# NidhiMishra/SR_object_detection

Hardware: AMD Instinct MI355X
Metric: images/sec YOLOv2 608x608 fp32 (higher is better)
Workload: dtype f32

## Files before the change

### include/y2_hip.h

```cpp
#ifndef Y2_HIP_H
#define Y2_HIP_H

#include <stddef.h>
#include <stdint.h>

#ifdef __cplusplus
extern "C" {
#endif

#define Y2H_OK            0
#define Y2H_EHIP         -1
#define Y2H_EINVAL       -2
#define Y2H_ENODEV       -3

typedef void *y2h_stream;
typedef void *y2h_event;
typedef void *y2h_graph;

enum { Y2H_ACT_LINEAR = 0, Y2H_ACT_LEAKY = 1, Y2H_ACT_LOGISTIC = 2, Y2H_ACT_RELU = 3,
       Y2H_ACT_RELIE = 4, Y2H_ACT_RAMP = 5, Y2H_ACT_TANH = 6, Y2H_ACT_PLSE = 7, Y2H_ACT_ELU = 8, Y2H_ACT_LOGGY = 9,
       Y2H_ACT_STAIR = 10, Y2H_ACT_HARDTAN = 11, Y2H_ACT_LHTAN = 12 };

int         y2h_device_count(void);
int         y2h_set_device(int dev);
// ... 49 lines not shown
    int activation;
    const float  *x;
    const float  *w_packed;
    const float  *w_ref;
    const float  *mean;
    const double *rinv;
    const float  *scale;
    const float  *bias;
    float        *y;
    float        *ws;
    size_t        ws_bytes;
    int           x_f16;
    int           y_f16;
    const float  *alpha;
    const float  *beta;
    int           tile_bm, tile_bn;
    int           ksplit;
    int           x_nchw;
} y2h_conv;

int y2h_conv_candidates(const y2h_conv *d, int *bm, int *bn, int *ks, int max);

int y2h_conv_first_layer_nchw_ok(const y2h_conv *d);

int y2h_conv_uses_mfma(const y2h_conv *d);
size_t y2h_conv_workspace_bytes(const y2h_conv *d);
int y2h_p8_stream_k_plan(long ntiles, int nk, long grid, int *sk_tiles, int *sk_wgs);
int y2h_sk_shares(long tiles, int nk, long G, int *out);
int y2h_sk_first(long tiles, int nk, long G, int *out);
int y2h_sk_walk(long tiles, int nk, long G, int *out, int max);
unsigned long y2h_stream_k_launches(void);
unsigned long y2h_tail_launches(void);
unsigned long y2h_xcd_order_launches(void);
unsigned long y2h_f32_stream_k_launches(void);
int y2h_conv_first_layer_ok(const y2h_conv *d);
int y2h_conv_stem_halo(const y2h_conv *d);
int y2h_conv_first_layer_f16_ok(const y2h_conv *d);
int y2h_conv_forward(const y2h_conv *d, int strict, y2h_stream s);
const char *y2h_conv_variant(const y2h_conv *d, int strict);

typedef struct y2h_wino {
    int eligible;
    int take;
    int bm, bn;
    long tiles, tiles_pad;
    size_t u_bytes;
    size_t v_bytes, m_bytes;
    double direct_cost, gemm_cost, wino_cost;
} y2h_wino;
int y2h_wino_plan(const y2h_conv *d, y2h_wino *out);
size_t y2h_wino_workspace_bytes(const y2h_conv *d);
int y2h_conv_wino_forward(const y2h_conv *d, y2h_stream s);
unsigned long y2h_wino_launches(void);

int y2h_maxpool(const float *x, int ldx, float *y, int ldy, int batch, int h, int w, int c,
                int size, int stride, int pad, int out_h, int out_w, y2h_stream s);
int y2h_reorg(const float *x, int ldx, float *y, int ldy, int batch, int h, int w, int c,
              int stride, int reverse, y2h_stream s);
int y2h_connected_ref(const float *x, long x_batch_stride, int ld, int hw, int c, const float *w_ref, float *y,
                      int outputs, int batch, int batch_normalize, int activation, const float *mean,
                      const double *rinv, const float *scale, const float *bias, y2h_stream s);
int y2h_detection_boxes(const float *pred, long pred_stride, int batch, int side, int num, int classes, int sqrt_flag,
                        int w, int h, float thresh, int only_objectness, float *boxes, float *probs, y2h_stream s);
int y2h_shortcut(const float *in, int ld_in, const float *add, int ld_add, float *out, int ld_out, int batch,
                 int w1, int h1, int c1, int w2, int h2, int c2, int activation, y2h_stream s);
int y2h_crop(const float *x, int ldx, float *y, int ldy, int batch, int h, int w, int c, int out_h, int out_w,
             int noadjust, int halo, y2h_stream s);
int y2h_batchnorm(const float *x, int ldx, float *y, int ldy, long pixels, int c, const float *mean, const double *rinv,
                  const float *scale, y2h_stream s);
int y2h_local(const float *x, int ldx, const float *w_packed, const float *bias_packed, float *y, int ldy, int batch,
              int h, int w, int c, int n, int size, int stride, int pad, int out_h, int out_w, int activation,
              int strict, y2h_stream s);
int y2h_binarize(const float *x, int ldx, float *y, long rows, int c, y2h_stream s);
int y2h_activate_array(float *x, int ld, long rows, int c, int activation, y2h_stream s);
int y2h_activate_copy(const float *x, int ldx, float *y, int ldy, long rows, int c, int activation, y2h_stream s);
int y2h_activate_copy_f16(const void *x, int ldx, void *y, int ldy, long rows, int c, int activation, y2h_stream s);
int y2h_lrn_fast_ok(int c, int size);
int y2h_lrn(const float *x, int ldx, float *y, int ldy, long pixels, int c, int size, float alpha, float beta, float kappa,
            int strict, y2h_stream s);
int y2h_lrn_f16(const void *x, int ldx, void *y, int ldy, long pixels, int c, int size, float alpha, float beta, float kappa,
                y2h_stream s);
int y2h_avgpool(const float *x, int ldx, float *y, int batch, int h, int w, int c, y2h_stream s);
int y2h_softmax_rows(const float *x, float *y, long rows, int n, float temp, y2h_stream s);
int y2h_softmax_tree_rows(const float *x, float *y, long rows, int n, float temp, int groups, const int *group_size,
                          const int *group_offset, const int *group_of, y2h_stream s);
int y2h_hierarchy_rows(float *rows, long ld, int nrows, int n, const int *parent, const int *order, const int *level_off,
                       int levels, const int *leaf, const int *row_mask, y2h_stream s);

int y2h_maxpool_f16(const void *x, int ldx, void *y, int ldy, int batch, int h, int w, int c,
                    int size, int stride, int pad, int out_h, int out_w, y2h_stream s);
int y2h_reorg_f16(const void *x, int ldx, void *y, int ldy, int batch, int h, int w, int c,
                  int stride, int reverse, y2h_stream s);
int y2h_copy_channels_f16(const void *src, int ld_src, void *dst, int ld_dst, int c, long npix, y2h_stream s);
int y2h_avgpool_f16(const void *x, int ldx, float *y, int batch, int h, int w, int c, y2h_stream s);
int y2h_nhwc_f16_to_nchw(const void *src, int ld, float *dst, int n, int c, int h, int w, y2h_stream s);
int y2h_nchw_to_nhwc4_halo_f16(const float *src, void *dst, int n, int c, int h, int w, y2h_stream s);
int y2h_f32_to_f16(const float *src, void *dst, long n, y2h_stream s);
int y2h_f16_to_f32(const void *src, float *dst, long n, y2h_stream s);

int y2h_connected_f16_plan(int rows, int inputs, int outputs, int forced, int *ranges, size_t *ws_bytes, int *bounds,
                           int max_bounds);
int y2h_connected_f16(const void *x, long ldx, const void *w, const float *alpha, const float *beta, void *y, int ldy,
                      int y_f16, int rows, int inputs, int outputs, int activation, int ranges, float *ws, size_t ws_bytes,
                      y2h_stream s);
int y2h_local_f16(const void *x, int ldx, const void *w_packed, const float *bias_packed, void *y, int ldy, int batch,
                  int h, int w, int c, int n, int size, int stride, int pad, int out_h, int out_w, int activation,
// ... 228 lines not shown
```

### sr_object_detection_amd/csrc/host/y2_arena.c

```c
#include <math.h>
#include <stdio.h>
#include <stdlib.h>
#include <string.h>
#include "y2_internal.h"
#include "y2_wino_rule.h"

static int owns_arena(const layer *l)
{
    return l->type == CONVOLUTIONAL || l->type == CONNECTED || l->type == LOCAL || l->type == BATCHNORM || is_recurrent(l);
}

void y2_bn_slots(size_t *off, int n, size_t *mean, size_t *scale, size_t *rinv)
{
    *mean = *off; *off = align_up(*off + n * sizeof(float), 64);
    *scale = *off; *off = align_up(*off + n * sizeof(float), 64);
    *rinv = *off; *off = align_up(*off + n * sizeof(double), 64);
}

void y2_fill_rinv(double *dst, const float *var, int n)
{
    int f;
    for (f = 0; f < n; ++f) dst[f] = 1.0 / (sqrt((double)var[f]) + (double).000001f);
}

static float xnor_filter_mean(const float *w, int K)
{
    float bmean = 0;
    int q;
    for (q = 0; q < K; ++q) bmean += fabs(w[q]);
    return bmean / K;
}

static unsigned short f32_to_f16_rne(float f)
{
    unsigned int x, sign, mant;
    int exp;
    memcpy(&x, &f, sizeof x);
    sign = (x >> 16) & 0x8000u;
    exp = (int)((x >> 23) & 0xff) - 127 + 15;
    mant = x & 0x7fffffu;
    if (((x >> 23) & 0xff) == 0xff) return (unsigned short)(sign | 0x7c00u | (mant ? 0x200u : 0));
    if (exp >= 31) return (unsigned short)(sign | 0x7c00u);
    if (exp <= 0) {
        unsigned int shift, half, rem;
        if (exp < -10) return (unsigned short)sign;
        mant |= 0x800000u;
        shift = (unsigned int)(14 - exp);
        half = mant >> shift;
        rem = mant & ((1u << shift) - 1);
        if (rem > (1u << (shift - 1)) || (rem == (1u << (shift - 1)) && (half & 1))) ++half;
        return (unsigned short)(sign | half);
    }
    {
        unsigned int half = ((unsigned int)exp << 10) | (mant >> 13), rem = mant & 0x1fffu;
        if (rem > 0x1000u || (rem == 0x1000u && (half & 1))) ++half;
        return (unsigned short)(sign | half);
    }
}

void y2_arena_layout(network *net)
{
    y2_engine *e = y2_engine_of(net);
    size_t off = 0;
    int i;
    for (i = 0; i < net->n; ++i) {
        const layer *l = &net->layers[i];
        y2_ldev *d = ld_of(l);
        const size_t wbytes = (size_t)l->n * l->size * l->size * l->c * sizeof(float);
        const int w_half = y2_half_weights(net, i);
        if (!owns_arena(l)) continue;
        if (l->type == BATCHNORM) { y2_bn_slots(&off, l->c, &d->off_mean, &d->off_scale, &d->off_rinv); continue; }
        if (is_recurrent(l)) { off = y2_rec_layout(d, l, off); continue; }
        if (l->type == LOCAL) {
            d->off_w_packed = off; off = align_up(off + (size_t)l->out_h * l->out_w * l->n * l->size * l->size * l->c * (w_half ? 2 : sizeof(float)), 256);
            d->off_bias = off; off = align_up(off + (size_t)l->outputs * sizeof(float), 64);
            continue;
        }
        d->off_w_packed = off; off = align_up(off + (d->wino ? (size_t)16 * l->n * l->c * sizeof(float) : w_half ? wbytes / 2 : wbytes), 256);
        if (d->has_w_ref) { d->off_w_ref = off; off = align_up(off + wbytes, 256); }
        d->off_bias = off; off = align_up(off + l->n * sizeof(float), 64);
        if (w_half) {
            d->off_alpha = off; off = align_up(off + l->n * sizeof(float), 64);
            d->off_beta = off; off = align_up(off + l->n * sizeof(float), 64);
        }
        if (l->batch_normalize) y2_bn_slots(&off, l->n, &d->off_mean, &d->off_scale, &d->off_rinv);
    }
    e->arena_need = off;
}

static uint64_t arena_signature(const network *net)
{
    const y2_engine *e = y2_engine_of(net);
    uint64_t sig = 1469598103934665603ull;
    int i, k;
#define SIG_MIX(v) do { uint64_t v_ = (uint64_t)(v); int b_; for (b_ = 0; b_ < 8; ++b_) { sig ^= (v_ >> (8 * b_)) & 0xff; sig *= 1099511628211ull; } } while (0)
    for (i = 0; i < net->n; ++i) {
        const layer *l = &net->layers[i];
        const y2_ldev *d = ld_of(l);
        if (!owns_arena(l)) continue;
        if (is_recurrent(l)) {
            for (k = 0; k < 3; ++k) { SIG_MIX(i); SIG_MIX(d->rd[k].off_w); SIG_MIX(d->rd[k].off_bias); SIG_MIX(d->rd[k].bn ? d->rd[k].off_rinv + 1 : 0); }
            continue;
        }
        SIG_MIX(i); SIG_MIX(d->off_w_packed); SIG_MIX(d->has_w_ref ? d->off_w_ref + 1 : 0); SIG_MIX(d->off_bias);
        SIG_MIX(d->uses_mfma); SIG_MIX(y2_half_weights(net, i));
        SIG_MIX(l->batch_normalize ? d->off_rinv + 1 : 0);
        if (d->wino) SIG_MIX(0x57494e4f);
    }
    SIG_MIX(e->strict); SIG_MIX(e->half); SIG_MIX(e->arena_need);
#undef SIG_MIX
    return sig;
}

int y2_arena_commit(network *net)
{
    y2_engine *e = y2_engine_of(net);
    const uint64_t sig = arena_signature(net);
    const int had_layout = e->arena_sig != 0;
    if (e->arena_need != e->arena_bytes || !e->arena) {
        if (e->arena) y2h_free(e->arena);
        e->arena = NULL;
        e->arena_bytes = e->arena_need;
        HIP_OR_ERR(y2h_malloc((void **)&e->arena, e->arena_need));
        e->arena_sig = 0;
    }
    if (sig == e->arena_sig) return 0;
    if (e->weights_external && had_layout) {
        e->weights_external = 0;
        y2_fail("the weight arena was filled from outside (y2_weights_resident) for another plan "
                "(strict / fp16 / fusion / size changed its layout): call y2_weights_arena() again and replicate the "
                "weights for the new plan");
        return -1;
    }
    if (!e->weights_external) e->weights_dirty = 1;
    e->arena_sig = sig;
    return 0;
}

static void pack_local(unsigned char *host, const y2_ldev *d, const layer *l, int w_half)
{
    const int locations = l->out_h * l->out_w, kk = l->size * l->size, K = kk * l->c;
    float *wp = (float *)(host + d->off_w_packed), *b = (float *)(host + d->off_bias);
    int loc, co, ci, t;
    for (loc = 0; loc < locations; ++loc)
        for (co = 0; co < l->n; ++co) {
            const float *src = l->weights + ((size_t)loc * l->n + co) * K;
            float *dst = wp + ((size_t)loc * l->n + co) * K;
            for (ci = 0; ci < l->c; ++ci)
                for (t = 0; t < kk; ++t) {
                    if (w_half) ((unsigned short *)wp)[((size_t)loc * l->n + co) * K + (size_t)t * l->c + ci] = f32_to_f16_rne(src[(size_t)ci * kk + t]);
                    else dst[(size_t)t * l->c + ci] = src[(size_t)ci * kk + t];
                }
            b[(size_t)loc * l->n + co] = l->biases[(size_t)co * locations + loc];
        }
}

static void pack_filters(float *wp, const network *net, int i, int w_half)
{
    const layer *l = &net->layers[i];
    const int K = l->size * l->size * l->c;
    int co, ci, kh, kw;
    if (l->type == CONNECTED) {
        const layer *pl = i > 0 ? &net->layers[y2_producer_of(net, i)] : NULL;
        const int hw = (pl && !y2_is_flat(net, y2_producer_of(net, i))) ? pl->out_h * pl->out_w : 1;
        const int C = K / (hw > 0 ? hw : 1);
        int pix;
        for (co = 0; co < l->n; ++co)
            for (ci = 0; ci < C; ++ci)
                for (pix = 0; pix < hw; ++pix) {
                    const size_t dst = (size_t)co * K + (size_t)pix * C + ci;
                    const float v = l->weights[(size_t)co * K + (size_t)ci * hw + pix];
                    if (w_half) ((unsigned short *)wp)[dst] = f32_to_f16_rne(v);
                    else wp[dst] = v;
                }
        return;
    }
    for (co = 0; co < l->n; ++co) {
        const float bmean = l->xnor ? xnor_filter_mean(l->weights + (size_t)co * K, K) : 0;
        for (ci = 0; ci < l->c; ++ci)
            for (kh = 0; kh < l->size; ++kh)
                for (kw = 0; kw < l->size; ++kw) {
                    const size_t dst = (size_t)co * K + (size_t)(kh * l->size + kw) * l->c + ci;
                    float v = l->weights[(((size_t)co * l->c + ci) * l->size + kh) * l->size + kw];
                    if (l->xnor) v = (v > 0) ? bmean : -bmean;
                    if (w_half) ((unsigned short *)wp)[dst] = f32_to_f16_rne(v);
                    else wp[dst] = v;
                }
    }
}

static void pack_wino(float *up, const layer *l)
{
    const size_t comp = (size_t)l->n * l->c;
    int co, ci, g;
    for (co = 0; co < l->n; ++co)
        for (ci = 0; ci < l->c; ++ci) {
            float u[16];
            y2_wino_filter(l->weights + ((size_t)co * l->c + ci) * 9, u);
            for (g = 0; g < 16; ++g) up[g * comp + (size_t)co * l->c + ci] = u[g];
        }
}

static void pack_dense(unsigned char *host, const network *net, int i)
{
    const layer *l = &net->layers[i];
    const y2_ldev *d = ld_of(l);
    const int K = l->size * l->size * l->c, w_half = y2_half_weights(net, i);
    int co, f, q;
    if (d->wino) pack_wino((float *)(host + d->off_w_packed), l);
    else pack_filters((float *)(host + d->off_w_packed), net, i, w_half);
    if (w_half) {
        float *al = (float *)(host + d->off_alpha), *be = (float *)(host + d->off_beta);
        for (f = 0; f < l->n; ++f) {
            double a = 1.0, bb = l->biases[f];
            if (l->batch_normalize) {
                a = (double)l->scales[f] / (sqrt((double)l->rolling_variance[f]) + (double).000001f);
                bb = (double)l->biases[f] - (double)l->rolling_mean[f] * a;
            }
            al[f] = (float)a; be[f] = (float)bb;
        }
    }
    if (d->has_w_ref) memcpy(host + d->off_w_ref, l->weights, (size_t)l->n * K * sizeof(float));
    if (d->has_w_ref && l->type == CONVOLUTIONAL && l->xnor) {
        float *wr = (float *)(host + d->off_w_ref);
        for (co = 0; co < l->n; ++co) {
            const float bmean = xnor_filter_mean(l->weights + (size_t)co * K, K);
            for (q = 0; q < K; ++q) wr[(size_t)co * K + q] = (l->weights[(size_t)co * K + q] > 0) ? bmean : -bmean;
        }
    }
    memcpy(host + d->off_bias, l->biases, l->n * sizeof(float));
    if (l->batch_normalize) {
        memcpy(host + d->off_mean, l->rolling_mean, l->n * sizeof(float));
        memcpy(host + d->off_scale, l->scales, l->n * sizeof(float));
        y2_fill_rinv((double *)(host + d->off_rinv), l->rolling_variance, l->n);
    }
}

int y2_upload_weights(network *net)
{
    y2_engine *e = y2_engine_of(net);
    unsigned char *host = NULL;
    int i;
    if (y2h_host_alloc((void **)&host, e->arena_bytes ? e->arena_bytes : 16) != 0) host = NULL;
    if (!host) { y2_fail("weight upload: no pinned host memory for %zu bytes: %s", e->arena_bytes, y2h_last_error()); return -1; }
    memset(host, 0, e->arena_bytes ? e->arena_bytes : 16);
    for (i = 0; i < net->n; ++i) {
        const layer *l = &net->layers[i];
        const y2_ldev *d = ld_of(l);
        if (!owns_arena(l)) continue;
        if (is_recurrent(l)) y2_rec_pack(host, d, l);
        else if (l->type == BATCHNORM) {
            memcpy(host + d->off_mean, l->rolling_mean, l->c * sizeof(float));
            memcpy(host + d->off_scale, l->scales, l->c * sizeof(float));
            y2_fill_rinv((double *)(host + d->off_rinv), l->rolling_variance, l->c);
        }
        else if (l->type == LOCAL) pack_local(host, d, l, y2_half_weights(net, i));
        else pack_dense(host, net, i);
    }
    if (y2h_memcpy_h2d(e->arena, host, e->arena_bytes, e->stream) != 0 || y2h_stream_sync(e->stream) != 0) {
        y2h_host_free(host);
        y2_fail("weight upload failed: %s", y2h_last_error());
        return -1;
// ... 37 lines not shown
```

### sr_object_detection_amd/csrc/host/y2_engine.c

```c
#include <math.h>
#include <stdio.h>
#include <stdlib.h>
#include <string.h>
#include "y2_internal.h"

void y2_drop_graphs(y2_engine *e)
{
    int k;
    for (k = 0; k < 4; ++k) {
        if (e->graphs[k]) y2h_graph_destroy(e->graphs[k]);
        e->graphs[k] = NULL; e->graph_srcs[k] = NULL;
    }
    e->graph = NULL; e->graph_src = NULL; e->graph_next = 0;
}

y2_engine *y2_engine_of(const network *net) { return net ? (y2_engine *)net->engine : NULL; }

int y2_engine_create(network *net)
{
    y2_engine *e = calloc(1, sizeof *e);
    int i;
    const char *st = getenv("Y2_STRICT");
    e->device = net->gpu_index;
    e->weights_dirty = 1;
// ... 142 lines not shown
    return 0;
}

static int forward_input(network *net, const float *d_input_nchw)
{
    y2_engine *e = y2_engine_of(net);
    const int misaligned = ((uintptr_t)d_input_nchw % 16) != 0;
    e->cur_input = d_input_nchw;
    if (y2_flat_input(net)) {
        if (misaligned && d_input_nchw != e->d_in_nchw) {
            HIP_OR_ERR(y2h_memcpy_d2d(e->d_in_nchw, d_input_nchw, e->in_floats * sizeof(float), e->stream));
            e->cur_input = e->d_in_nchw;
        }
        return 0;
    }
    switch (e->in_form) {
    case Y2_IN_NCHW:
        if (!e->half || !misaligned) break;
        if (d_input_nchw != e->d_in_nchw) HIP_OR_ERR(y2h_memcpy_d2d(e->d_in_nchw, d_input_nchw, e->in_floats * sizeof(float), e->stream));
        e->cur_input = e->d_in_nchw;
        break;
    case Y2_IN_NHWC4_HALO_F16:
        HIP_OR_ERR(y2h_nchw_to_nhwc4_halo_f16(d_input_nchw, e->d_in_nhwc, net->batch, net->c, net->h, net->w, e->stream));
        break;
    case Y2_IN_NHWC_HALO:
        HIP_OR_ERR(y2h_nchw_to_nhwc_halo(d_input_nchw, e->d_in_nhwc, net->batch, net->c, net->h, net->w, net->c, e->in_halo_px, e->stream));
        break;
    case Y2_IN_NHWC:
        HIP_OR_ERR(y2h_nchw_to_nhwc(d_input_nchw, e->d_in_nhwc, net->batch, net->c, net->h, net->w, net->c, e->stream));
        break;
    }
    return 0;
}

int y2_activate_after(y2_engine *e, ACTIVATION a, float *y, int ld, long rows, int n)
{
    if (!y2_act_in_kernel(a)) HIP_OR_ERR(y2h_activate_array(y, ld, rows, n, y2_act_code(a), e->stream));
    return 0;
}

static int forward_convolutional(network *net, int i, const float *x, int ldx)
{
    y2_engine *e = y2_engine_of(net);
    const layer *l = &net->layers[i];
    const y2_ldev *d = ld_of(l);
    y2h_conv c;
    if (l->xnor) {
        const float *px; int pld;
        if (i == 0) { px = e->d_in_nhwc; pld = net->c; }
        else { const y2_ldev *p = ld_of(&net->layers[i - 1]); px = p->out; pld = p->out_ld; }
        HIP_OR_ERR(y2h_binarize(px, pld, d->d_bin, (long)l->batch * l->h * l->w, l->c, e->stream));
    }
    y2_conv_desc(net, i, &c, x, ldx);
    if (d->wino) HIP_OR_ERR(y2h_conv_wino_forward(&c, e->stream));
    else HIP_OR_ERR(y2h_conv_forward(&c, e->strict, e->stream));
    return y2_activate_after(e, l->activation, d->out, d->out_ld, (long)l->batch * l->out_h * l->out_w, l->out_c);
}

static int forward_route(network *net, int i)
{
    y2_engine *e = y2_engine_of(net);
    const layer *l = &net->layers[i];
    const y2_ldev *d = ld_of(l);
    int k, choff = 0;
    if (l->n < 2 || !d->copy_mask) return 0;
    for (k = 0; k < l->n; ++k) {
        const layer *src = &net->layers[l->input_layers[k]];
        const y2_ldev *sd = ld_of(src);
        if ((d->copy_mask & (1u << k)) && d->out_half)
            HIP_OR_ERR(y2h_copy_channels_f16(sd->out, sd->out_ld, (unsigned short *)d->out + choff, d->out_ld, src->out_c,
                                             (long)l->batch * l->out_h * l->out_w, e->stream));
        else if (d->copy_mask & (1u << k))
            HIP_OR_ERR(y2h_copy_channels(sd->out, sd->out_ld, d->out + choff, d->out_ld, src->out_c,
                                         (long)l->batch * l->out_h * l->out_w, e->stream));
        choff += src->out_c;
    }
    return 0;
}

static int forward_region(network *net, int i, const float *x, int ldx)
{
    y2_engine *e = y2_engine_of(net);
    const layer *l = &net->layers[i];
    y2_ldev *d = ld_of(l);
    const tree *t = l->softmax_tree;
    if (e->det_overlap && e->det_pending == 1 && i == e->out_layer && !e->capturing) HIP_OR_ERR(y2h_stream_wait_event(e->stream, e->ev_det));
    d->tree_best_valid = 0;
    if (t && d->d_tree_best && !e->det_overlap) d->tree_best_valid = 1;
    if (t)
        HIP_OR_ERR(y2h_region_forward_tree(x, ldx, d->d_region, l->batch, l->h * l->w, l->n, l->classes, l->coords, t->groups,
                                           d->d_tree_gsize, d->d_tree_goff, d->d_tree_parent, d->d_tree_order, d->d_tree_loff,
                                           d->tree_levels, d->tree_best_valid ? d->d_tree_best : NULL,
                                           e->strict ? 0 : Y2H_REGION_FAST_EXP, e->stream));
    else
        HIP_OR_ERR(y2h_region_forward(x, ldx, d->d_region, l->batch, l->h * l->w, l->n, l->classes, l->coords, l->softmax,
                                      0, d->d_tree_gsize, d->d_tree_goff, e->stream));
    return 0;
}

static int forward_connected(network *net, int i, const float *x, int ldx)
{
    y2_engine *e = y2_engine_of(net);
    const layer *l = &net->layers[i];
    const y2_ldev *d = ld_of(l);
    y2h_conv c;
    y2_conv_desc(net, i, &c, x, ldx);
    if (d->conn_ranges && !e->strict) {
// ... 548 lines not shown
```

### sr_object_detection_amd/csrc/host/y2_internal.h

```cpp
#ifndef Y2_INTERNAL_H
#define Y2_INTERNAL_H

#include <stddef.h>
#include <stdint.h>
#include "sr_yolo2.h"
#include "y2_hip.h"

typedef struct y2_ldev {
    struct y2_engine *eng;
    int index;
    float *out;
    int out_ld;
    float *out_alloc;
    size_t out_floats;
    int placed_in;
    int alias_of;
    unsigned copy_mask;
    size_t off_w_packed, off_w_ref, off_bias, off_mean, off_scale, off_rinv;
    int has_w_ref;
    int uses_mfma;
    int wino;
    int fused_pool;
    int fused_into;
    int out_half;
    size_t off_alpha, off_beta;
    char kname[80];
    int tile_bm, tile_bn, ksplit;
    int conn_ranges;
    float *d_anchors;
    int *d_tree_block, *h_tree_block;
    size_t tree_block_ints;
    int *d_tree_parent, *d_tree_gsize, *d_tree_goff, *d_map;
    int *d_tree_order, *d_tree_loff;
    int tree_levels;
    int *d_tree_group, *d_tree_leaf, *h_tree_leaf;
    float *d_tree_best;
    int tree_best_valid;
    float *d_region;
    float *d_flat;
    float *d_halo;
    int halo_px;
    float *d_bin;
    const char *kernel;
    struct { size_t off_w, off_bias, off_mean, off_scale, off_rinv; int n, k, bn; ACTIVATION act; int form; } rd[3];
    float *d_state;
    float *d_proj;
    float *d_hist;
    float *d_zf;
    float *d_tmp;
} y2_ldev;

enum { Y2_REC_REF = 0, Y2_REC_SKINNY = 1, Y2_REC_MFMA = 2 };

enum { Y2_LR_CONSTANT = 0, Y2_LR_STEP, Y2_LR_EXP, Y2_LR_POLY, Y2_LR_STEPS, Y2_LR_SIG, Y2_LR_RANDOM };
typedef struct {
    int policy, step, burn_in, num_steps, adam;
    float scale, gamma, power;
    int *steps;
    float *scales;
} y2_lr_schedule;

typedef struct y2_engine {
    int device;
    y2h_stream stream;
    int strict;
    int timing;
    int fusion, built_fusion;
    int half, built_half;
    int autotune, built_autotune;
    int in_form;
    const float *cur_input;
    int in_halo_px;
    y2h_event ev_out;
    int out_pending;
// ... 163 lines not shown
```

### sr_object_detection_amd/csrc/host/y2_plan.c

```c
#include <math.h>
#include <stdio.h>
#include <stdlib.h>
#include <pthread.h>
#include <string.h>
#include "y2_internal.h"

void y2_free_plan(network *net)
{
    y2_engine *e = y2_engine_of(net);
    int i;
    if (!e) return;
    for (i = 0; i < net->n; ++i) {
        y2_ldev *d = ld_of(&net->layers[i]);
        if (!d) continue;
        y2h_free(d->out_alloc); d->out_alloc = NULL; d->out = NULL;
        y2h_free(d->d_region); d->d_region = NULL;
        y2h_free(d->d_flat); d->d_flat = NULL;
        y2h_free(d->d_halo); d->d_halo = NULL; d->halo_px = 0;
        y2h_free(d->d_bin); d->d_bin = NULL;
        y2h_free(d->d_state); d->d_state = NULL;
        y2h_free(d->d_proj); d->d_proj = NULL;
        y2h_free(d->d_hist); d->d_hist = NULL;
        y2h_free(d->d_zf); d->d_zf = NULL;
        y2h_free(d->d_tmp); d->d_tmp = NULL;
        d->placed_in = -1; d->alias_of = -1; d->copy_mask = 0;
        d->fused_pool = 0; d->fused_into = -1;
        d->out_half = 0;
        d->wino = 0;
        d->tile_bm = d->tile_bn = d->ksplit = 0;
        d->conn_ranges = 0;
    }
    y2_drop_graphs(e);
    y2h_free(e->d_in_nchw); e->d_in_nchw = NULL;
    y2h_free(e->d_in_nhwc); e->d_in_nhwc = NULL;
    y2h_free(e->d_out_nchw); e->d_out_nchw = NULL;
    y2h_free(e->d_ws); e->d_ws = NULL; e->ws_bytes = 0;
    y2h_free(e->d_u8); e->d_u8 = NULL; e->u8_cap = 0;
    y2h_free(e->d_planes); e->d_planes = NULL; e->planes_cap = 0;
    y2h_free(e->d_rtmp); e->d_rtmp = NULL; e->rtmp_cap = 0;
    if (e->reg_pending) { y2h_event_sync(e->ev_reg); e->reg_pending = 0; }
    y2h_free(e->d_reg); e->d_reg = NULL; e->reg_cap = 0;
    y2h_free(e->d_boxes); e->d_boxes = NULL;
    y2h_free(e->d_probs); e->d_probs = NULL;
    y2h_free(e->d_probs_nms); e->d_probs_nms = NULL;
    y2h_free(e->d_records); e->d_records = NULL;
    y2h_free(e->d_counts); e->d_counts = NULL;
    y2h_free(e->d_class_counts); e->d_class_counts = NULL;
    y2h_free(e->d_best); e->d_best = NULL;
    y2h_free(e->d_mean_ring); e->d_mean_ring = NULL; e->mean_els = 0; e->mean_index = 0;
    y2h_host_free(e->h_records); e->h_records = NULL;
    y2h_host_free(e->h_counts); e->h_counts = NULL;
    e->built = 0;
}

static int producer_can_place(const layer *l)
{
    return l->type == CONVOLUTIONAL || l->type == MAXPOOL || l->type == REORG;
}

int y2_act_code(ACTIVATION a)
{
    switch (a) {
    case LINEAR: return Y2H_ACT_LINEAR;
    case LEAKY: return Y2H_ACT_LEAKY;
    case LOGISTIC: return Y2H_ACT_LOGISTIC;
    case RELU: return Y2H_ACT_RELU;
    case RELIE: return Y2H_ACT_RELIE;
    case RAMP: return Y2H_ACT_RAMP;
    case TANH: return Y2H_ACT_TANH;
    case PLSE: return Y2H_ACT_PLSE;
    case ELU: return Y2H_ACT_ELU;
    case LOGGY: return Y2H_ACT_LOGGY;
    case STAIR: return Y2H_ACT_STAIR;
    case HARDTAN: return Y2H_ACT_HARDTAN;
    case LHTAN: return Y2H_ACT_LHTAN;
    }
    return -1;
}
int y2_act_in_kernel(ACTIVATION a) { const int c = y2_act_code(a); return c >= 0 && c <= Y2H_ACT_RELU; }
int y2_act_for_kernel(ACTIVATION a) { return y2_act_in_kernel(a) ? y2_act_code(a) : Y2H_ACT_LINEAR; }
static const char *act_name(ACTIVATION a)
// ... 105 lines not shown
    }
}

int y2_half_weights(const network *net, int i)
{
    const y2_ldev *pd;
    if (i <= 0) return 0;
    pd = ld_of(&net->layers[net->layers[i].type == CONNECTED ? y2_producer_of(net, i) : i - 1]);
    if (!pd->out_half) return 0;
    return !(net->layers[i].type == CONVOLUTIONAL && pd->d_halo);
}

static int conn_forced_ranges(void)
{
    const char *ks = getenv("Y2_CONN_KSPLIT");
    return (ks && atoi(ks) > 0) ? atoi(ks) : 0;
}

static int upload_small(void **dst, const void *src, size_t bytes, y2h_stream s)
{
    if (*dst) { y2h_free(*dst); *dst = NULL; }
    if (y2h_malloc(dst, bytes) != 0) return -1;
    if (y2h_memcpy_h2d(*dst, src, bytes, s) != 0) return -1;
    return y2h_stream_sync(s);
}

static int grow_workspace(y2_engine *e, size_t need)
{
    if (need <= e->ws_bytes) return 0;
    y2h_free(e->d_ws); e->d_ws = NULL; e->ws_bytes = 0;
    HIP_OR_ERR(y2h_malloc((void **)&e->d_ws, need));
    e->ws_bytes = need;
    return 0;
}

static int plan_workspace(network *net)
{
    y2_engine *e = y2_engine_of(net);
    size_t need = y2_rec_workspace_bytes(net);
    int i;
    for (i = 0; i < net->n; ++i) {
        y2h_conv c;
        const float *x; int ldx;
        size_t b;
        if ((net->layers[i].type != CONVOLUTIONAL && net->layers[i].type != CONNECTED) || e->strict) continue;
        if (ld_of(&net->layers[i])->conn_ranges) {
            const layer *l = &net->layers[i];
            if (y2h_connected_f16_plan(l->batch, l->inputs, l->outputs, ld_of(l)->conn_ranges, NULL, &b, NULL, 0) == 0 && b > need) need = b;
            continue;
        }
        y2_input_view(net, i, &x, &ldx);
        conv_query(net, i, &c, x, ldx);
        b = ld_of(&net->layers[i])->wino ? y2h_wino_workspace_bytes(&c) : y2h_conv_workspace_bytes(&c);
        if (b > need) need = b;
    }
    return grow_workspace(e, need);
}

typedef struct { int batch, h, w, c, n, size, stride, pool, bm, bn, ks; } tune_entry;
static tune_entry g_tuned[256];
static int g_ntuned = 0;
static pthread_mutex_t g_tuned_mu = PTHREAD_MUTEX_INITIALIZER;

static int autotune_layers(network *net)
{
    y2_engine *e = y2_engine_of(net);
    const int keep_timing = e->timing;
    int i, k, a;
    size_t need = 0;
    for (i = 0; i < net->n; ++i) {
        const layer *l = &net->layers[i];
        y2_ldev *d = ld_of(l);
        y2h_conv c;
        const float *x; int ldx, n, bm[64], bn[64], ks[64];
        if (l->type != CONVOLUTIONAL || !d->uses_mfma || l->xnor || d->wino) continue;
        y2_input_view(net, i, &x, &ldx);
        y2_conv_desc(net, i, &c, x, ldx);
        n = y2h_conv_candidates(&c, bm, bn, ks, 64);
        for (a = 0; a < n; ++a) {
            size_t b = (size_t)ks[a] * l->batch * l->out_h * l->out_w * l->out_c * sizeof(float);
            if (ks[a] > 1 && b > need) need = b;
        }
    }
    if (grow_workspace(e, need) != 0) return -1;
    if (y2h_memset(e->d_in_nchw, 0, e->in_floats * sizeof(float), e->stream) != 0) { y2_fail("autotune: %s", y2h_last_error()); return -1; }
    e->timing = 1;
    for (i = 0; i < net->n; ++i) {
        layer *l = &net->layers[i];
        y2_ldev *d = ld_of(l);
        y2h_conv c;
        const float *x; int ldx, n, hit = 0, bm[64], bn[64], ks[64], best = 0;
        float best_ms = 0.f;
        if (l->type != CONVOLUTIONAL || !d->uses_mfma || l->xnor || d->wino) continue;
        y2_input_view(net, i, &x, &ldx);
        y2_conv_desc(net, i, &c, x, ldx);
        pthread_mutex_lock(&g_tuned_mu);
        for (k = 0; k < g_ntuned && !hit; ++k) {
            const tune_entry *t = &g_tuned[k];
            if (t->batch == c.batch && t->h == c.h && t->w == c.w && t->c == c.c && t->n == c.n && t->size == c.size &&
                t->stride == c.stride && t->pool == c.fuse_maxpool2) { d->tile_bm = t->bm; d->tile_bn = t->bn; d->ksplit = t->ks; hit = 1; }
        }
        pthread_mutex_unlock(&g_tuned_mu);
        if (!hit && 2.0 * l->batch * l->out_h * l->out_w * (double)l->n * l->size * l->size * l->c > 40e9) continue;
        if (!hit) {
            c.tile_bm = c.tile_bn = c.ksplit = 0;
            n = y2h_conv_candidates(&c, bm, bn, ks, 64);
            if (n < 0) { e->timing = keep_timing; y2_fail("autotune of layer %d failed (%d): %s", i, n, y2h_last_error()); return -1; }
            if (n == 0) continue;
            for (a = 0; a < n; ++a) {
                float ms = 0.f, m2 = 0.f;
                int rep;
                d->tile_bm = bm[a]; d->tile_bn = bn[a]; d->ksplit = ks[a];
                for (rep = 0; rep < 2; ++rep) {
                    if (y2_enqueue_forward(net, e->d_in_nchw) != 0) { e->timing = keep_timing; return -1; }
                    if (y2h_event_elapsed_ms(e->ev[i], e->ev[i + 1], &m2) != 0) { e->timing = keep_timing; y2_fail("autotune: %s", y2h_last_error()); return -1; }
                    ms = (rep == 0 || m2 < ms) ? m2 : ms;
                }
                if (getenv("Y2_AUTOTUNE_LOG"))
                    fprintf(stderr, "autotune layer %2d %3dx%-3d c%-4d n%-5d k%d%s: %3dx%-3d ks%-2d %.4f ms%s\n", i, l->h, l->w, l->c, l->n, l->size,
                            c.fuse_maxpool2 ? "+pool" : "", bm[a], bn[a], ks[a], ms, a == 0 ? "  (model)" : "");
                if (a == 0) ms *= 0.98f;
                if (a == 0 || ms < best_ms) { best_ms = ms; best = a; }
            }
            d->tile_bm = bm[best]; d->tile_bn = bn[best]; d->ksplit = ks[best];
            pthread_mutex_lock(&g_tuned_mu);
            if (g_ntuned < (int)(sizeof g_tuned / sizeof g_tuned[0])) {
                tune_entry *t = &g_tuned[g_ntuned++];
                t->batch = c.batch; t->h = c.h; t->w = c.w; t->c = c.c; t->n = c.n; t->size = c.size; t->stride = c.stride;
                t->pool = c.fuse_maxpool2; t->bm = d->tile_bm; t->bn = d->tile_bn; t->ks = d->ksplit;
            }
            pthread_mutex_unlock(&g_tuned_mu);
        }
        y2_conv_desc(net, i, &c, x, ldx);
        d->kernel = y2h_conv_variant(&c, 0);
        if (d->fused_pool) { snprintf(d->kname, sizeof d->kname, "%s+maxpool2", d->kernel); d->kernel = d->kname; }
    }
    e->timing = keep_timing;
    HIP_OR_ERR(y2h_stream_sync(e->stream));
    return 0;
}

static int autotune_allowed(const y2_engine *e) { return e->autotune && !e->strict && !e->arena_pending; }

int y2_softmax_tree_check(const network *net)
{
    int i, g, j, count;
// ... 476 lines not shown
            const char *form = getenv("Y2_CONN_F16");
            const int tile_ok = y2h_conv_uses_mfma(&c) && strncmp(y2h_conv_variant(&c, 0), "conv_mfma_f16", 13) == 0;
            int tile = tile_ok && l->batch > 16;
            if (form && strcmp(form, "skinny") == 0) tile = 0;
            if (form && strcmp(form, "mfma") == 0) tile = tile_ok;
            d->uses_mfma = tile;
            d->has_w_ref = 0;
            if (tile) { d->kernel = y2h_conv_variant(&c, 0); continue; }
            if (y2h_connected_f16_plan(l->batch, l->inputs, l->outputs, conn_forced_ranges(), &d->conn_ranges, NULL, NULL, 0) != 0) {
                y2_fail("fp16 mode: layer %d (connected): %d inputs x %d outputs cannot be planned", i, l->inputs, l->outputs);
                return -1;
            }
            snprintf(d->kname, sizeof d->kname, d->conn_ranges > 1 ? "connected_f16+ksplit%d" : "connected_f16", d->conn_ranges);
            d->kernel = d->kname;
            continue;
        }
        d->uses_mfma = !e->strict && y2h_conv_uses_mfma(&c);
        if (d->fused_pool && !d->uses_mfma) {
            y2_ldev *md = ld_of(&net->layers[i + 1]);
            d->fused_pool = 0; md->fused_into = -1; md->kernel = "maxpool_nhwc";
            if (alloc_activations(d, l) != 0) return -1;
            conv_query(net, i, &c, x, ldx);
        }
        d->has_w_ref = !d->uses_mfma;
        d->kernel = y2h_conv_variant(&c, e->strict);
        if (l->type == CONNECTED && !d->uses_mfma) d->kernel = "connected_ref";
        if (d->fused_pool) { snprintf(d->kname, sizeof d->kname, "%s+maxpool2", d->kernel); d->kernel = d->kname; }
    }
    return 0;
}

static int plan_wino(network *net)
{
    y2_engine *e = y2_engine_of(net);
    int i;
    if (e->strict || e->half) return 0;
    for (i = 0; i < net->n; ++i) {
        layer *l = &net->layers[i];
        y2_ldev *d = ld_of(l);
        y2h_conv c;
        y2h_wino w;
        const float *x; int ldx;
        if (l->type != CONVOLUTIONAL || !d->uses_mfma || l->xnor) continue;
        y2_input_view(net, i, &x, &ldx);
        conv_query(net, i, &c, x, ldx);
        if (y2h_wino_plan(&c, &w) != 0 || !w.take) continue;
        d->wino = 1;
        snprintf(d->kname, sizeof d->kname, "conv_wino_f32_%dx%dx32%s", w.bm, w.bn, d->fused_pool ? "+maxpool2" : "");
        d->kernel = d->kname;
    }
    return 0;
}

static int plan_timing_events(network *net)
{
    y2_engine *e = y2_engine_of(net);
    int i;
    if (e->n_ev == net->n + 1) return 0;
    if (e->ev) { for (i = 0; i < e->n_ev; ++i) y2h_event_destroy(e->ev[i]); free(e->ev); }
    e->n_ev = net->n + 1;
    e->ev = calloc(e->n_ev, sizeof(y2h_event));
    for (i = 0; i < e->n_ev; ++i) HIP_OR_ERR(y2h_event_create(&e->ev[i]));
    return 0;
}

int y2_engine_build(network *net)
{
    y2_engine *e = y2_engine_of(net);
    if (plan_checks(net) != 0) return -1;
    y2_free_plan(net);
    if (plan_batches(net) != 0 || plan_routes(net) != 0 || plan_pool_fusion(net) != 0 || plan_half(net) != 0 ||
        plan_activations(net) != 0 || plan_input_copies(net) != 0 || plan_input(net) != 0 || plan_output(net) != 0 ||
        plan_head_constants(net) != 0 || plan_conv_kernels(net) != 0 || plan_wino(net) != 0) return -1;
    y2_arena_layout(net);
    if (plan_workspace(net) != 0 || y2_arena_commit(net) != 0 || plan_timing_events(net) != 0) return -1;
    e->built = 1;
    e->built_batch = net->batch; e->built_w = net->w; e->built_h = net->h; e->built_strict = e->strict;
    e->built_fusion = e->fusion;
    e->built_half = e->half;
    if (!e->weights_external) e->arena_pending = 0;
    e->built_autotune = e->arena_pending ? 0 : e->autotune;
    if (e->weights_dirty && !e->weights_external && y2_upload_weights(net) != 0) return -1;
    if (autotune_allowed(e)) {
        if (autotune_layers(net) != 0 || plan_workspace(net) != 0) { e->built = 0; return -1; }
    }
    return 0;
}
```

Measured before the change: 2726.

## Add specialized Winograd F(2x2,3x3) kernel for 32-input-channel 3x3 convolutions

Adds a new persistent Winograd conv kernel for 3x3 stride-1 layers with exactly 32 input channels (the YOLOv2 second conv layer at 304x304), using 8x16 output patches staged in double-buffered LDS with fp32 MFMA over transformed tiles, fused BN/leaky/maxpool epilogue. Planner selects it when enough patches exist, packs transformed filters into a custom MFMA-friendly layout, and skips autotune/workspace for those layers. Aims to cut multiply count and avoid the im2col/gemm path for this large early layer; risks numerical differences from Winograd and depends on kernel being better than the tuned direct path.

```diff
diff --git a/include/y2_hip.h b/include/y2_hip.h
--- a/include/y2_hip.h
+++ b/include/y2_hip.h
@@ -125,6 +125,17 @@
 size_t y2h_wino_workspace_bytes(const y2h_conv *d);
 int y2h_conv_wino_forward(const y2h_conv *d, y2h_stream s);
 unsigned long y2h_wino_launches(void);
+
+typedef struct y2h_winos {
+    int eligible;
+    int take;
+    int form;
+    long patches;
+    size_t u_bytes;
+} y2h_winos;
+int y2h_winos_plan(const y2h_conv *d, y2h_winos *out);
+int y2h_conv_winos_forward(const y2h_conv *d, y2h_stream s);
+unsigned long y2h_winos_launches(void);
 
 int y2h_maxpool(const float *x, int ldx, float *y, int ldy, int batch, int h, int w, int c,
                 int size, int stride, int pad, int out_h, int out_w, y2h_stream s);
diff --git a/include/y2_winos_rule.h b/include/y2_winos_rule.h
--- /dev/null
+++ b/include/y2_winos_rule.h
@@ -0,0 +1,32 @@
+#ifndef Y2_WINOS_RULE_H
+#define Y2_WINOS_RULE_H
+
+#include <stddef.h>
+
+#define Y2_WINOS_MIN_PATCHES 1024L
+#define Y2_WINOS_PATCH_H 8
+#define Y2_WINOS_PATCH_W 16
+
+static inline int y2_winos_shape_ok(int size, int stride, int pad, int c, int n, int h, int w, int out_h, int out_w, int pool,
+                                    int x_f16, int y_f16, int x_halo, int x_nchw, int ldx)
+{
+    (void)pool;
+    if (x_f16 || y_f16 || x_halo || x_nchw) return 0;
+    if (size != 3 || stride != 1 || pad != 1 || out_h != h || out_w != w) return 0;
+    if (c != 32 || n < 4 || n > 64 || n % 4 != 0 || ldx % 4 != 0) return 0;
+    if (h <= 0 || w <= 0 || h % Y2_WINOS_PATCH_H != 0 || w % Y2_WINOS_PATCH_W != 0) return 0;
+    return 1;
+}
+
+static inline long y2_winos_patches(int batch, int h, int w) { return (long)batch * (h / Y2_WINOS_PATCH_H) * (w / Y2_WINOS_PATCH_W); }
+
+static inline int y2_winos_wins(long patches) { return patches >= Y2_WINOS_MIN_PATCHES; }
+
+static inline size_t y2_winos_u_floats(int n) { return (size_t)((n + 31) / 32) * 4 * 16 * 64 * 4; }
+static inline size_t y2_winos_u_index(int co, int ci, int i, int j)
+{
+    const size_t fq = (size_t)(co / 32), lane = (size_t)(32 * ((ci % 8) / 4) + co % 32), kk = (size_t)(4 * j + ci / 8);
+    return (((fq * 4 + (size_t)i) * 16 + kk) * 64 + lane) * 4 + (size_t)(ci % 4);
+}
+
+#endif
diff --git a/sr_object_detection_amd/csrc/host/y2_arena.c b/sr_object_detection_amd/csrc/host/y2_arena.c
--- a/sr_object_detection_amd/csrc/host/y2_arena.c
+++ b/sr_object_detection_amd/csrc/host/y2_arena.c
@@ -4,6 +4,7 @@
 #include <string.h>
 #include "y2_internal.h"
 #include "y2_wino_rule.h"
+#include "y2_winos_rule.h"
 
 static int owns_arena(const layer *l)
 {
@@ -76,7 +77,7 @@
             d->off_bias = off; off = align_up(off + (size_t)l->outputs * sizeof(float), 64);
             continue;
         }
-        d->off_w_packed = off; off = align_up(off + (d->wino ? (size_t)16 * l->n * l->c * sizeof(float) : w_half ? wbytes / 2 : wbytes), 256);
+        d->off_w_packed = off; off = align_up(off + (d->winos ? y2_winos_u_floats(l->n) * sizeof(float) : d->wino ? (size_t)16 * l->n * l->c * sizeof(float) : w_half ? wbytes / 2 : wbytes), 256);
         if (d->has_w_ref) { d->off_w_ref = off; off = align_up(off + wbytes, 256); }
         d->off_bias = off; off = align_up(off + l->n * sizeof(float), 64);
         if (w_half) {
@@ -106,6 +107,7 @@
         SIG_MIX(d->uses_mfma); SIG_MIX(y2_half_weights(net, i));
         SIG_MIX(l->batch_normalize ? d->off_rinv + 1 : 0);
         if (d->wino) SIG_MIX(0x57494e4f);
+        if (d->winos) SIG_MIX(0x57494e53);
     }
     SIG_MIX(e->strict); SIG_MIX(e->half); SIG_MIX(e->arena_need);
 #undef SIG_MIX
@@ -201,13 +203,26 @@
         }
 }
 
+static void pack_winos(float *up, const layer *l)
+{
+    int co, ci, g;
+    memset(up, 0, y2_winos_u_floats(l->n) * sizeof(float));
+    for (co = 0; co < l->n; ++co)
+        for (ci = 0; ci < l->c; ++ci) {
+            float u[16];
+            y2_wino_filter(l->weights + ((size_t)co * l->c + ci) * 9, u);
+            for (g = 0; g < 16; ++g) up[y2_winos_u_index(co, ci, g >> 2, g & 3)] = u[g];
+        }
+}
+
 static void pack_dense(unsigned char *host, const network *net, int i)
 {
     const layer *l = &net->layers[i];
     const y2_ldev *d = ld_of(l);
     const int K = l->size * l->size * l->c, w_half = y2_half_weights(net, i);
     int co, f, q;
-    if (d->wino) pack_wino((float *)(host + d->off_w_packed), l);
+    if (d->winos) pack_winos((float *)(host + d->off_w_packed), l);
+    else if (d->wino) pack_wino((float *)(host + d->off_w_packed), l);
     else pack_filters((float *)(host + d->off_w_packed), net, i, w_half);
     if (w_half) {
         float *al = (float *)(host + d->off_alpha), *be = (float *)(host + d->off_beta);
diff --git a/sr_object_detection_amd/csrc/host/y2_engine.c b/sr_object_detection_amd/csrc/host/y2_engine.c
--- a/sr_object_detection_amd/csrc/host/y2_engine.c
+++ b/sr_object_detection_amd/csrc/host/y2_engine.c
@@ -218,7 +218,8 @@
         HIP_OR_ERR(y2h_binarize(px, pld, d->d_bin, (long)l->batch * l->h * l->w, l->c, e->stream));
     }
     y2_conv_desc(net, i, &c, x, ldx);
-    if (d->wino) HIP_OR_ERR(y2h_conv_wino_forward(&c, e->stream));
+    if (d->winos) HIP_OR_ERR(y2h_conv_winos_forward(&c, e->stream));
+    else if (d->wino) HIP_OR_ERR(y2h_conv_wino_forward(&c, e->stream));
     else HIP_OR_ERR(y2h_conv_forward(&c, e->strict, e->stream));
     return y2_activate_after(e, l->activation, d->out, d->out_ld, (long)l->batch * l->out_h * l->out_w, l->out_c);
 }
diff --git a/sr_object_detection_amd/csrc/host/y2_internal.h b/sr_object_detection_amd/csrc/host/y2_internal.h
--- a/sr_object_detection_amd/csrc/host/y2_internal.h
+++ b/sr_object_detection_amd/csrc/host/y2_internal.h
@@ -20,6 +20,7 @@
     int has_w_ref;
     int uses_mfma;
     int wino;
+    int winos;
     int fused_pool;
     int fused_into;
     int out_half;
diff --git a/sr_object_detection_amd/csrc/host/y2_plan.c b/sr_object_detection_amd/csrc/host/y2_plan.c
--- a/sr_object_detection_amd/csrc/host/y2_plan.c
+++ b/sr_object_detection_amd/csrc/host/y2_plan.c
@@ -27,6 +27,7 @@
         d->fused_pool = 0; d->fused_into = -1;
         d->out_half = 0;
         d->wino = 0;
+        d->winos = 0;
         d->tile_bm = d->tile_bn = d->ksplit = 0;
         d->conn_ranges = 0;
     }
@@ -238,6 +239,7 @@
         y2_input_view(net, i, &x, &ldx);
         conv_query(net, i, &c, x, ldx);
         b = ld_of(&net->layers[i])->wino ? y2h_wino_workspace_bytes(&c) : y2h_conv_workspace_bytes(&c);
+        if (ld_of(&net->layers[i])->winos) b = 0;
         if (b > need) need = b;
     }
     return grow_workspace(e, need);
@@ -259,7 +261,7 @@
         y2_ldev *d = ld_of(l);
         y2h_conv c;
         const float *x; int ldx, n, bm[64], bn[64], ks[64];
-        if (l->type != CONVOLUTIONAL || !d->uses_mfma || l->xnor || d->wino) continue;
+        if (l->type != CONVOLUTIONAL || !d->uses_mfma || l->xnor || d->wino || d->winos) continue;
         y2_input_view(net, i, &x, &ldx);
         y2_conv_desc(net, i, &c, x, ldx);
         n = y2h_conv_candidates(&c, bm, bn, ks, 64);
@@ -277,7 +279,7 @@
         y2h_conv c;
         const float *x; int ldx, n, hit = 0, bm[64], bn[64], ks[64], best = 0;
         float best_ms = 0.f;
-        if (l->type != CONVOLUTIONAL || !d->uses_mfma || l->xnor || d->wino) continue;
+        if (l->type != CONVOLUTIONAL || !d->uses_mfma || l->xnor || d->wino || d->winos) continue;
         y2_input_view(net, i, &x, &ldx);
         y2_conv_desc(net, i, &c, x, ldx);
         pthread_mutex_lock(&g_tuned_mu);
@@ -860,6 +862,28 @@
     return 0;
 }
 
+static int plan_winos(network *net)
+{
+    y2_engine *e = y2_engine_of(net);
+    int i;
+    if (e->strict || e->half) return 0;
+    for (i = 0; i < net->n; ++i) {
+        layer *l = &net->layers[i];
+        y2_ldev *d = ld_of(l);
+        y2h_conv c;
+        y2h_winos w;
+        const float *x; int ldx;
+        if (l->type != CONVOLUTIONAL || !d->uses_mfma || l->xnor || d->wino) continue;
+        y2_input_view(net, i, &x, &ldx);
+        conv_query(net, i, &c, x, ldx);
+        if (y2h_winos_plan(&c, &w) != 0 || !w.take) continue;
+        d->winos = 1;
+        snprintf(d->kname, sizeof d->kname, "conv_winos_f32_c%d%s", w.form, d->fused_pool ? "+maxpool2" : "");
+        d->kernel = d->kname;
+    }
+    return 0;
+}
+
 static int plan_timing_events(network *net)
 {
     y2_engine *e = y2_engine_of(net);
@@ -879,7 +903,7 @@
     y2_free_plan(net);
     if (plan_batches(net) != 0 || plan_routes(net) != 0 || plan_pool_fusion(net) != 0 || plan_half(net) != 0 ||
         plan_activations(net) != 0 || plan_input_copies(net) != 0 || plan_input(net) != 0 || plan_output(net) != 0 ||
-        plan_head_constants(net) != 0 || plan_conv_kernels(net) != 0 || plan_wino(net) != 0) return -1;
+        plan_head_constants(net) != 0 || plan_conv_kernels(net) != 0 || plan_wino(net) != 0 || plan_winos(net) != 0) return -1;
     y2_arena_layout(net);
     if (plan_workspace(net) != 0 || y2_arena_commit(net) != 0 || plan_timing_events(net) != 0) return -1;
     e->built = 1;
diff --git a/sr_object_detection_amd/csrc/y2_winos.hip b/sr_object_detection_amd/csrc/y2_winos.hip
--- /dev/null
+++ b/sr_object_detection_amd/csrc/y2_winos.hip
@@ -0,0 +1,250 @@
+#include "y2_conv_shared.hpp"
+#include "y2_winos_rule.h"
+#include <string.h>
+
+namespace {
+
+constexpr int WS_PW = 18, WS_PH = 10, WS_PIX_B = 144, WS_ROW_B = WS_PW * WS_PIX_B, WS_BUF_B = WS_PH * WS_ROW_B;
+constexpr int WS_NCH = WS_PH * WS_PW * 8;
+constexpr int WS_NP = (WS_NCH + 511) / 512;
+constexpr int WS_EX_P = 36;
+constexpr int WS_EX_COMP = 32 * WS_EX_P;
+constexpr int WS_EX_FQ = 8 * WS_EX_COMP;
+constexpr int WS_CONST_B = 64 * (3 * 4 + 8);
+constexpr size_t WS_LDS = (size_t)2 * WS_BUF_B + (size_t)2 * WS_EX_FQ * 4 + WS_CONST_B;
+
+__device__ __forceinline__ int ws_tile(int li)
+{
+    const int q = li >> 2;
+    return 16 * (__builtin_popcount(q) & 1) + ((q >> 1) << 2) + (li & 3);
+}
+
+__device__ __forceinline__ f32x4 flip(f32x4 v, unsigned neg)
+{
+    u32x4 b = __builtin_bit_cast(u32x4, v);
+    b ^= neg;
+    return __builtin_bit_cast(f32x4, b);
+}
+
+template <bool POOL, bool FAST>
+__global__ __launch_bounds__(512, 2) void conv_winos_c32_kernel(ConvK a)
+{
+    extern __shared__ __attribute__((aligned(16))) unsigned char ws_smem[];
+    const int t = threadIdx.x, lane = t & 63, li = lane & 31, lh = lane >> 5;
+    const int wv = __builtin_amdgcn_readfirstlane(t >> 6);
+    const int fq = wv & 1, wi = wv >> 1;
+    const bool BN_ = FAST ? true : (bool)a.bn;
+    const int ACT_ = FAST ? (int)Y2H_ACT_LEAKY : a.act;
+    const __amdgpu_buffer_rsrc_t xr = __builtin_amdgcn_make_buffer_rsrc((void *)a.x, 0, a.xbytes, 0x00020000);
+    const __amdgpu_buffer_rsrc_t wr = __builtin_amdgcn_make_buffer_rsrc((void *)a.w, 0, a.wbytes, 0x00020000);
+    const __amdgpu_buffer_rsrc_t yr = __builtin_amdgcn_make_buffer_rsrc((void *)a.y, 0, a.ybytes, 0x00020000);
+
+    float *ex = (float *)(ws_smem + 2 * WS_BUF_B);
+    float *c_mean = ex + 2 * WS_EX_FQ, *c_scale = c_mean + 64, *c_bias = c_scale + 64;
+    double *c_rinv = (double *)(c_bias + 64);
+    if (t < 64) {
+        float mean = 0.f, scale = 1.f, bias = 0.f;
+        double rinv = 1.0;
+        if (t < a.Cout) {
+            bias = a.bias[t];
+            if (BN_) { mean = a.mean[t]; rinv = a.rinv[t]; scale = a.scale[t]; }
+        }
+        c_mean[t] = mean; c_scale[t] = scale; c_bias[t] = bias; c_rinv[t] = rinv;
+    }
+
+    f32x4 bu[16];
+#pragma unroll
+    for (int kk = 0; kk < 16; ++kk) {
+        const unsigned off = 32 * fq < a.Cout ? (unsigned)((((fq * 4 + wi) * 16 + kk) * 64 + lane) * 16) : a.wbytes;
+        bu[kk] = __builtin_bit_cast(f32x4, __builtin_amdgcn_raw_buffer_load_b128(wr, off, 0, 0));
+    }
+
+    const int ldxB = a.ldx * 4;
+    int s_lds[WS_NP], s_rel[WS_NP], s_yx[WS_NP];
+#pragma unroll
+    for (int p = 0; p < WS_NP; ++p) {
+        const int q = t + 512 * p;
+        const int pixel = q >> 3, part = q & 7;
+        const int py = pixel / WS_PW, px = pixel - py * WS_PW;
+        s_lds[p] = py * WS_ROW_B + px * WS_PIX_B + ((px >> 2) & 1) * 16 + part * 16;
+        s_rel[p] = ((py - 1) * a.W + (px - 1)) * ldxB + part * 16;
+        s_yx[p] = q < WS_NCH ? (py << 8) | px : -1;
+    }
+    const int blocks_x = a.W >> 4, bpi = (a.H >> 3) * blocks_x;
+    const int nblocks = a.batch * bpi;
+    u32x4 sreg[WS_NP];
+    auto load_patch = [&](int blk) {
+        const int n = blk / bpi, rem = blk - n * bpi;
+        const int oy0 = (rem / blocks_x) << 3, ox0 = (rem - (rem / blocks_x) * blocks_x) << 4;
+        const unsigned base = (unsigned)((n * a.H + oy0) * a.W + ox0) * (unsigned)ldxB;
+#pragma unroll
+        for (int p = 0; p < WS_NP; ++p) {
+            const int iy = oy0 - 1 + (s_yx[p] >> 8), ix = ox0 - 1 + (s_yx[p] & 255);
+            const bool ok = s_yx[p] >= 0 && iy >= 0 && iy < a.H && ix >= 0 && ix < a.W;
+            sreg[p] = __builtin_amdgcn_raw_buffer_load_b128(xr, ok ? base + (unsigned)s_rel[p] : a.xbytes, 0, 0);
+        }
+    };
+    auto store_patch = [&](int buf) {
+#pragma unroll
+        for (int p = 0; p < WS_NP; ++p)
+            if (s_yx[p] >= 0) *(u32x4 *)(ws_smem + buf * WS_BUF_B + s_lds[p]) = sreg[p];
+    };
+
+    const int ra = wi == 0 ? 0 : wi == 2 ? 2 : 1;
+    const int rb = wi == 0 ? 2 : wi == 1 ? 2 : wi == 2 ? 1 : 3;
+    const unsigned neg = wi == 1 ? 0u : 0x80000000u;
+    const int aty = ws_tile(li) >> 3, atx = ws_tile(li) & 7;
+    const int a_off0 = 2 * aty * WS_ROW_B + 2 * atx * WS_PIX_B + ((atx >> 1) & 1) * 16 + lh * 16;
+    const int a_off1 = 2 * aty * WS_ROW_B + (2 * atx + 2) * WS_PIX_B + (((atx + 1) >> 1) & 1) * 16 + lh * 16;
+    const int otx = lane >> 3, cq = 32 * fq + (lane & 7) * 4;
+    const bool fok = cq < a.Cout;
+    const float *exr = ex + fq * WS_EX_FQ + (wi * 8 + otx) * WS_EX_P + (lane & 7) * 4;
+    float *exw = ex + fq * WS_EX_FQ + (wi * 2) * WS_EX_COMP + li;
+    float *exw_even = exw + 16 * lh * WS_EX_P, *exw_odd = exw + 16 * (1 - lh) * WS_EX_P;
+    const int Hp = a.H >> 1, Wp = a.W >> 1;
+
+    int blk = blockIdx.x, cur = 0;
+    if (blk < nblocks) { load_patch(blk); store_patch(0); }
+    __syncthreads();
+    for (; blk < nblocks; blk += gridDim.x, cur ^= 1) {
+        const int next = blk + gridDim.x;
+        if (next < nblocks) load_patch(next);
+        const unsigned char *ap0 = ws_smem + cur * WS_BUF_B + a_off0, *ap1 = ws_smem + cur * WS_BUF_B + a_off1;
+        f32x16 M[4];
+#pragma unroll
+        for (int j = 0; j < 4; ++j)
+#pragma unroll
+            for (int r = 0; r < 16; ++r) M[j][r] = 0.f;
+#pragma unroll
+        for (int g = 0; g < 4; ++g) {
+            f32x4 tc[4];
+#pragma unroll
+            for (int c = 0; c < 4; ++c) {
+                const unsigned char *ap = c < 2 ? ap0 + c * WS_PIX_B : ap1 + (c - 2) * WS_PIX_B;
+                const f32x4 da = *(const f32x4 *)(ap + ra * WS_ROW_B + g * 32);
+                const f32x4 db = *(const f32x4 *)(ap + rb * WS_ROW_B + g * 32);
+                tc[c] = da + flip(db, neg);
+            }
+            f32x4 v[4];
+            v[0] = tc[0] - tc[2]; v[1] = tc[1] + tc[2]; v[2] = tc[2] - tc[1]; v[3] = tc[1] - tc[3];
+#pragma unroll
+            for (int s4 = 0; s4 < 4; ++s4)
+#pragma unroll
+                for (int j = 0; j < 4; ++j)
+                    M[j] = __builtin_amdgcn_mfma_f32_32x32x2f32(v[j][s4], bu[4 * j + g][s4], M[j], 0, 0, 0);
+        }
+        const f32x16 S0 = (M[0] + M[1]) + M[2], S1 = (M[1] - M[2]) - M[3];
+        __syncthreads();
+#pragma unroll
+        for (int r = 0; r < 16; ++r) {
+            float *e = ((__builtin_popcount(r >> 2) & 1) ? exw_odd : exw_even) + (4 * (r >> 2) + (r & 3)) * WS_EX_P;
+            e[0] = S0[r];
+            e[WS_EX_COMP] = S1[r];
+        }
+        if (next < nblocks) store_patch(cur ^ 1);
+        __syncthreads();
+
+        f32x4 Y[2][2];
+#pragma unroll
+        for (int b = 0; b < 2; ++b) {
+            const f32x4 s0 = *(const f32x4 *)(exr + (0 + b) * WS_EX_COMP), s1 = *(const f32x4 *)(exr + (2 + b) * WS_EX_COMP);
+            const f32x4 s2 = *(const f32x4 *)(exr + (4 + b) * WS_EX_COMP), s3 = *(const f32x4 *)(exr + (6 + b) * WS_EX_COMP);
+            Y[0][b] = (s0 + s1) + s2;
+            Y[1][b] = (s1 - s2) - s3;
+        }
+        const f32x4 mean = *(const f32x4 *)(c_mean + cq), scale = *(const f32x4 *)(c_scale + cq), bias = *(const f32x4 *)(c_bias + cq);
+        double rinv[4];
+#pragma unroll
+        for (int q = 0; q < 4; ++q) rinv[q] = c_rinv[cq + q];
+        const int n = blk / bpi, rem = blk - n * bpi;
+        const int oy0 = (rem / blocks_x) << 3, ox0 = (rem - (rem / blocks_x) * blocks_x) << 4;
+        if (POOL) {
+            f32x4 o;
+#pragma unroll
+            for (int q = 0; q < 4; ++q)
+                o[q] = epilogue(pool_pick(Y[0][0][q], Y[0][1][q], Y[1][0][q], Y[1][1][q], !BN_ || scale[q] >= 0.f),
+                                BN_, mean[q], rinv[q], scale[q], bias[q], ACT_);
+            const unsigned prow = (unsigned)((n * Hp + (oy0 >> 1) + wi) * Wp + (ox0 >> 1) + otx);
+            const unsigned idx = prow * (unsigned)a.ldy + (unsigned)cq;
+            if (a.vec_store) __builtin_amdgcn_raw_buffer_store_b128(__builtin_bit_cast(u32x4, o), yr, fok ? idx * 4u : 0xffffffffu, 0, 0);
+            else if (fok) {
+#pragma unroll
+                for (int q = 0; q < 4; ++q) a.y[(size_t)idx + q] = o[q];
+            }
+        } else {
+#pragma unroll
+            for (int ya = 0; ya < 2; ++ya)
+#pragma unroll
+                for (int xb = 0; xb < 2; ++xb) {
+                    f32x4 o;
+#pragma unroll
+                    for (int q = 0; q < 4; ++q) o[q] = epilogue(Y[ya][xb][q], BN_, mean[q], rinv[q], scale[q], bias[q], ACT_);
+                    const unsigned prow = (unsigned)((n * a.H + oy0 + 2 * wi + ya) * a.W + ox0 + 2 * otx + xb);
+                    const unsigned idx = prow * (unsigned)a.ldy + (unsigned)cq;
+                    if (a.vec_store) __builtin_amdgcn_raw_buffer_store_b128(__builtin_bit_cast(u32x4, o), yr, fok ? idx * 4u : 0xffffffffu, 0, 0);
+                    else if (fok) {
+#pragma unroll
+                        for (int q = 0; q < 4; ++q) a.y[(size_t)idx + q] = o[q];
+                    }
+                }
+        }
+    }
+}
+
+}
+
+extern "C" int y2h_winos_plan(const y2h_conv *d, y2h_winos *out)
+{
+    if (!d || !out) return Y2H_EINVAL;
+    memset(out, 0, sizeof *out);
+    int mode = -1;
+    if (const char *f = getenv("Y2_WINOS")) mode = atoi(f) != 0 ? 1 : 0;
+    if (!y2_winos_shape_ok(d->size, d->stride, d->pad, d->c, d->n, d->h, d->w, d->out_h, d->out_w, d->fuse_maxpool2, d->x_f16, d->y_f16,
+                           d->x_halo, d->x_nchw, d->ldx)) return Y2H_OK;
+    if (d->ldy < d->n || d->tile_bm || d->ksplit > 1 || getenv("Y2_CONV_TILE")) return Y2H_OK;
+    if (((uintptr_t)d->x | (uintptr_t)d->w_packed) % 16 != 0 || !d->w_packed) return Y2H_OK;
+    const double xbytes = (double)d->batch * d->h * d->w * d->ldx * 4.0;
+    const double ybytes = (double)d->batch * d->h * d->w * (d->fuse_maxpool2 ? 0.25 : 1.0) * d->ldy * 4.0;
+    if (xbytes >= 4294967000.0 || ybytes >= 4294967000.0) return Y2H_OK;
+    out->eligible = 1;
+    out->form = 32;
+    out->patches = y2_winos_patches(d->batch, d->h, d->w);
+    out->u_bytes = y2_winos_u_floats(d->n) * sizeof(float);
+    out->take = mode >= 0 ? mode : y2_winos_wins(out->patches);
+    return Y2H_OK;
+}
+
+static unsigned long g_winos_launches = 0;
+extern "C" unsigned long y2h_winos_launches(void) { return g_winos_launches; }
+
+extern "C" int y2h_conv_winos_forward(const y2h_conv *d, y2h_stream s)
+{
+    if (!d || !d->x || !d->y || !d->bias || !d->w_packed) return Y2H_EINVAL;
+    if (d->batch_normalize && (!d->mean || !d->rinv || !d->scale)) return Y2H_EINVAL;
+    y2h_winos w;
+    if (y2h_winos_plan(d, &w) != Y2H_OK || !w.take || w.form != 32) return Y2H_EINVAL;
+    ConvK a;
+    memset(&a, 0, sizeof a);
+    a.x = d->x; a.y = d->y; a.w = d->w_packed;
+    a.mean = d->mean; a.rinv = d->rinv; a.scale = d->scale; a.bias = d->bias;
+    a.H = d->h; a.W = d->w; a.Cin = d->c; a.ldx = d->ldx; a.Cout = d->n; a.ldy = d->ldy;
+    a.K = 9 * d->c;
+    a.bn = d->batch_normalize; a.act = d->activation;
+    a.size = 3; a.stride = 1; a.pad = 1; a.out_h = d->out_h; a.out_w = d->out_w; a.batch = d->batch;
+    a.pool = d->fuse_maxpool2 ? 1 : 0;
+    a.npix = d->batch * d->h * d->w;
+    a.xbytes = (unsigned)((size_t)d->batch * d->h * d->w * d->ldx * 4);
+    a.wbytes = (unsigned)w.u_bytes;
+    a.ybytes = (unsigned)((size_t)(a.pool ? a.npix / 4 : a.npix) * d->ldy * 4);
+    a.vec_store = d->ldy % 4 == 0 && (uintptr_t)d->y % 16 == 0;
+    const bool fast = d->batch_normalize && d->activation == Y2H_ACT_LEAKY;
+    void (*fn)(ConvK) = a.pool ? (fast ? conv_winos_c32_kernel<true, true> : conv_winos_c32_kernel<true, false>)
+                               : (fast ? conv_winos_c32_kernel<false, true> : conv_winos_c32_kernel<false, false>);
+    Y2H_CHECK(y2h_lds_limit((const void *)fn, WS_LDS));
+    long grid = w.patches < 256 ? w.patches : 256;
+    if (const char *g = getenv("Y2_CONV_GRID")) { if (atol(g) > 0 && atol(g) < grid) grid = atol(g); }
+    hipLaunchKernelGGL(fn, dim3((unsigned)grid), dim3(512), WS_LDS, S(s), a);
+    Y2H_LAUNCH_CHECK();
+    ++g_winos_launches;
+    return Y2H_OK;
+}
```

New measurement: 2785, median of 6. 2.2% higher.
